# ecmwf/anemoi-graphs

Hardware: NVIDIA B200
Metric: O1280->ico7 graph edges/sec (CutOff encoder + MultiScale processor + KNN-3 decoder + EdgeLength/EdgeDirection) (higher is better)
Workload: dtype f32 filter + f64 decisions, int32 indices

## Files before the change

anemoi_graphs_b200/_build.py:

```python

from __future__ import annotations

import os
import shutil
import subprocess
import sys
from pathlib import Path

PKG = Path(__file__).resolve().parent
CSRC = PKG / "csrc"
LIB_DIR = PKG / "lib"
LIB_PATH = LIB_DIR / "libagx_b200.so"
OBJ_DIR = LIB_DIR / "obj"
SOURCES = ["agx_util.cu", "agx_index.cu", "agx_knn.cu", "agx_radius.cu", "agx_attrs.cu", "agx_mesh.cu", "agx_hex.cu", "agx_voronoi.cu", "agx_concat.cu", "agx_postprocess.cu"]
NVCC_FLAGS = [
    "-gencode", "arch=compute_100a,code=sm_100a",
    "-lineinfo", "-O3", "-std=c++17",
    "-Xcompiler", "-fPIC",
    "-Xcompiler", "-fvisibility=default",
]
LINK_FLAGS = ["-gencode", "arch=compute_100a,code=sm_100a", "--shared", "-cudart", "static"]


def find_nvcc() -> str:
    for cand in (os.environ.get("NVCC"), shutil.which("nvcc"), "/usr/local/cuda/bin/nvcc"):
        if cand and Path(cand).exists():
            return cand
    raise RuntimeError("nvcc not found (set NVCC=/path/to/nvcc)")


def is_stale() -> bool:
    if not LIB_PATH.exists():
        return True
    built = LIB_PATH.stat().st_mtime
    deps = [CSRC / s for s in SOURCES] + list(CSRC.glob("*.cuh")) + [PKG.parent / "include" / "agx_b200.h"]
    return any(d.stat().st_mtime > built for d in deps)


def build(force: bool = False, verbose: bool = False) -> Path:
    if not force and not is_stale():
        return LIB_PATH
    LIB_DIR.mkdir(exist_ok=True)
    OBJ_DIR.mkdir(exist_ok=True)
    nvcc = find_nvcc()
    headers = list(CSRC.glob("*.cuh")) + [PKG.parent / "include" / "agx_b200.h"]
    newest_header = max(h.stat().st_mtime for h in headers)
    jobs = []
    for src in SOURCES:
        obj = OBJ_DIR / (src + ".o")
        if not force and obj.exists() and obj.stat().st_mtime > max((CSRC / src).stat().st_mtime, newest_header):
            continue
        cmd = [nvcc, *NVCC_FLAGS, "-c", "-o", str(obj), str(CSRC / src)]
        if verbose:
            cmd[1:1] = ["-Xptxas", "-v"]
            print(" ".join(cmd))
        jobs.append((src, subprocess.Popen(cmd, stdout=subprocess.PIPE, stderr=subprocess.PIPE, text=True)))
    for src, proc in jobs:
        out, err = proc.communicate()
        if proc.returncode != 0:
            for _, other in jobs:
                if other.poll() is None:
                    other.kill()
            raise RuntimeError(f"nvcc failed on {src}:\n{out}\n{err}")
        if verbose:
            print(err)
    tmp = LIB_PATH.with_suffix(".so.tmp")
    cmd = [nvcc, *LINK_FLAGS, "-o", str(tmp), *[str(OBJ_DIR / (s + ".o")) for s in SOURCES]]
    res = subprocess.run(cmd, capture_output=True, text=True)
    if res.returncode != 0:
        raise RuntimeError(f"link failed:\n{res.stdout}\n{res.stderr}")
    os.replace(tmp, LIB_PATH)
    return LIB_PATH


if __name__ == "__main__":
    path = build(force="--force" in sys.argv, verbose="-v" in sys.argv)
    print(path)
```

anemoi_graphs_b200/_cabi.py:

```python

from __future__ import annotations

import ctypes
from ctypes import POINTER, c_char_p, c_double, c_int, c_int32, c_int64, c_void_p
from pathlib import Path

import torch

LIB_PATH = Path(__file__).resolve().parent / "lib" / "libagx_b200.so"

ABI_VERSION = 3
AGX_OK = 0
AGX_ERR_CUDA = -1
AGX_ERR_ARG = -2
AGX_ERR_UNSUPPORTED = -3
AGX_ERR_OVERFLOW = -4

NORM_CODES = {None: 0, "l1": 1, "l2": 2, "unit-max": 3, "unit-range": 4, "unit-std": 5}

SIGNATURES = {
    "agx_last_error": (c_char_p, []),
    "agx_abi_version": (c_int, []),
    "agx_launch_count": (c_int64, []),
    "agx_index_build": (c_int, [c_void_p, c_int64, c_int, c_int, c_double, c_void_p, POINTER(c_void_p)]),
    "agx_index_free": (c_int, [c_void_p, c_void_p]),
    "agx_index_info": (c_int, [c_void_p, POINTER(c_int64), POINTER(c_int)]),
    "agx_search_vectors": (c_int, [c_void_p, c_int64, c_void_p, c_void_p]),
    "agx_knn": (
        c_int,
        [c_void_p, c_void_p, c_int64, c_int, c_double, c_void_p, c_void_p, c_int64, c_void_p, c_void_p, c_void_p],
    ),
    "agx_knn_flagged": (
        c_int,
        [c_void_p, c_void_p, c_int64, c_int, c_double, c_void_p, c_void_p, c_int64, c_void_p, c_void_p, c_void_p, c_void_p],
    ),
    "agx_knn_redecide": (c_int, [c_void_p, c_void_p, c_int64, c_int, c_double, c_void_p, c_void_p, c_void_p]),
    "agx_knn_redecide_ranked": (
        c_int,
        [c_void_p, c_void_p, c_int64, c_int, c_double, c_void_p, c_void_p, c_void_p, c_void_p, c_void_p],
    ),
    "agx_knn_redecide_list": (
        c_int,
        [c_void_p, c_void_p, c_int64, c_int, c_double, c_void_p, c_void_p, c_void_p, c_void_p, c_void_p, c_void_p],
    ),
    "agx_compact_flags": (c_int, [c_void_p, c_int64, c_void_p, c_void_p, c_void_p]),
    "agx_set_query_order_mode": (None, [c_int]),
    "agx_last_query_order": (c_int, []),
    "agx_radius_count": (c_int, [c_void_p, c_void_p, c_int64, c_double, c_void_p, c_void_p]),
    "agx_exclusive_scan": (c_int, [c_void_p, c_int64, c_void_p, POINTER(c_int64), c_void_p]),
    "agx_radius_fill": (c_int, [c_void_p, c_void_p, c_int64, c_double, c_void_p, c_void_p, c_void_p, c_int64, c_void_p, c_void_p]),
    "agx_max_positive": (c_int, [c_void_p, c_int64, POINTER(c_double), POINTER(c_int64), c_void_p]),
    "agx_host_reference_rdist": (c_int, [c_void_p, c_void_p, c_int64, c_int, POINTER(c_double)]),
    "agx_order_resolve": (c_int, [c_void_p, c_void_p, c_int64, c_void_p, c_void_p, c_void_p, c_void_p, c_void_p]),
    "agx_gate_supported": (c_int, []),
    "agx_gate_wait": (c_int, [c_void_p, c_void_p]),
    "agx_gate_open": (c_int, [c_void_p, c_void_p]),
    "agx_mark_nodes": (c_int, [c_void_p, c_int64, c_int64, c_void_p, c_void_p]),
    "agx_relabel_nodes": (c_int, [c_void_p, c_int64, c_void_p, c_void_p]),
    "agx_restrict_flags": (
        c_int,
        [c_void_p, c_void_p, c_int64, c_void_p, c_int64, c_void_p, c_int64, c_void_p, c_void_p, c_double, c_void_p, c_void_p],
    ),
    "agx_sort_edges": (c_int, [c_void_p, c_void_p, c_int64, c_int64, c_int64, c_int, c_void_p, c_void_p]),
    "agx_gather_edge_columns": (
        c_int,
        [c_int, POINTER(c_void_p), POINTER(c_void_p), POINTER(c_int64), c_void_p, c_int64, c_void_p],
    ),
    "agx_set_output_maps": (None, [c_void_p, c_void_p]),
    "agx_concat_edges": (
        c_int,
        [c_void_p, c_void_p, c_int64, c_void_p, c_void_p, c_int64, c_int64, c_int64, c_void_p, POINTER(c_int64), c_void_p],
    ),
    "agx_relabel_rows": (c_int, [POINTER(c_void_p), POINTER(c_int64), c_int, c_void_p, c_void_p]),
    "agx_node_tables": (c_int, [c_void_p, c_int64, c_void_p, c_void_p, c_void_p]),
    "agx_edge_attrs": (
        c_int,
        [c_void_p, c_void_p, c_int64, c_void_p, c_void_p, c_void_p, c_void_p, c_int, c_int, c_void_p, c_int, c_int,
         c_void_p, c_void_p, c_int, c_void_p],
    ),
    "agx_edge_attrs_workspace": (c_int64, []),
    "agx_edge_attrs_stats": (
        c_int,
        [c_void_p, c_void_p, c_int64, c_void_p, c_void_p, c_void_p, c_void_p, c_int, c_int, c_int, c_void_p, c_void_p,
         c_void_p, c_void_p, c_void_p],
    ),
    "agx_edge_attrs_stats_flagged": (
        c_int,
        [c_void_p, c_void_p, c_int64, c_void_p, c_void_p, c_void_p, c_void_p, c_int, c_int, c_int, c_void_p, c_void_p,
         c_void_p, c_void_p, c_void_p, c_int, c_int, c_void_p],
    ),
    "agx_edge_attrs_stats_list": (
        c_int,
        [c_void_p, c_void_p, c_int64, c_int, c_void_p, c_void_p, c_void_p, c_void_p, c_void_p, c_void_p, c_int, c_int,
         c_int, c_void_p, c_void_p, c_void_p, c_void_p, c_void_p],
    ),
    "agx_edge_attrs_apply": (
        c_int,
        [c_void_p, c_void_p, c_int64, c_void_p, c_void_p, c_void_p, c_void_p, c_int, c_int, c_void_p, c_int, c_int,
         c_void_p, c_void_p, c_int, c_int64, c_int, c_void_p, c_void_p],
    ),
    "agx_icosphere": (c_int, [c_int, c_void_p, c_void_p, c_void_p, c_void_p]),
    "agx_multiscale_tri_count": (
        c_int,
        [c_int, c_void_p, POINTER(c_int32), c_int, c_int, c_void_p, c_void_p, c_void_p, c_void_p, c_void_p],
    ),
    "agx_multiscale_scratch_per_node": (c_int64, [c_int, c_int]),
    "agx_multiscale_tri_count_mapped": (
        c_int,
        [c_int, c_void_p, POINTER(c_int32), c_int, c_int, c_int64, c_void_p, c_void_p, c_void_p, c_void_p, c_void_p],
    ),
    "agx_multiscale_tri_fill": (c_int, [c_int64, c_void_p, c_void_p, c_void_p, c_int64, c_void_p, c_void_p, c_void_p]),
    "agx_voronoi_areas": (
        c_int,
        [c_void_p, c_int64, c_void_p, c_int, c_int, c_void_p, c_int64, c_double, c_void_p, c_void_p, c_void_p],
    ),
    "agx_voronoi_areas_small": (c_int, [c_void_p, c_int64, c_void_p, c_int64, c_double, c_void_p, c_void_p, c_void_p]),
    "agx_healpix_nodes": (c_int, [c_int, c_void_p, c_void_p]),
    "agx_hex_num_cells": (c_int64, [c_int]),
    "agx_hex_cells": (c_int, [c_int, c_void_p, c_void_p, c_void_p]),
    "agx_hex_adjacency": (c_int, [c_void_p, c_void_p, c_int64, c_void_p, c_void_p, c_void_p]),
    "agx_multiscale_adj_count": (
        c_int,
        [c_int, POINTER(c_void_p), POINTER(c_void_p), POINTER(c_void_p), POINTER(c_void_p), c_int, c_int, c_int64,
         c_void_p, c_void_p, c_void_p],
    ),
}

_lib = None


class AgxError(RuntimeError):
    """A CUDA-side failure reported by libagx_b200."""


def load_library(path: Path | None = None) -> ctypes.CDLL:
    global _lib
    if _lib is not None and path is None:
        return _lib
    p = Path(path) if path is not None else LIB_PATH
    if not p.exists():
        raise RuntimeError(
            f"{p} is missing: the CUDA extension has not been built. Run `python -m anemoi_graphs_b200._build` "
            "(needs nvcc). This package has no CPU fallback."
        )
    lib = ctypes.CDLL(str(p))
    for name, (restype, argtypes) in SIGNATURES.items():
        fn = getattr(lib, name)
        fn.restype = restype
        fn.argtypes = argtypes
    if lib.agx_abi_version() != ABI_VERSION:
        raise RuntimeError(f"{p}: ABI version {lib.agx_abi_version()} != {ABI_VERSION}; rebuild the library")
    if path is None:
        _lib = lib
    return lib


def require_cuda() -> None:
    if not torch.cuda.is_available():
        raise RuntimeError(
            "anemoi_graphs_b200 needs a CUDA device (B200, sm_100a); there is no CPU fallback for the "
            "edge-construction path."
        )


def check(rc: int) -> None:
    if rc == AGX_OK:
        return
    msg = load_library().agx_last_error().decode(errors="replace")
    if rc == AGX_ERR_ARG:
        raise ValueError(msg)
    if rc == AGX_ERR_UNSUPPORTED:
        raise NotImplementedError(msg)
    raise AgxError(f"libagx_b200 error {rc}: {msg}")


def ptr(t: torch.Tensor | None) -> int | None:
    if t is None:
        return None
    assert t.is_cuda and t.is_contiguous(), "C-ABI buffers must be contiguous CUDA tensors"
    return t.data_ptr()


def current_stream() -> int:
    return torch.cuda.current_stream().cuda_stream


def launch_count() -> int:
    return int(load_library().agx_launch_count())
```

anemoi_graphs_b200/device.py:

```python

from __future__ import annotations

import contextlib
import os
from dataclasses import dataclass, field

import torch

from . import _cabi

_defer_depth = 0
_pending: list[torch.cuda.Event] = []
_works: dict[int, list] = {}
_resident = False


def set_resident(flag: bool) -> bool:
    global _resident
    prev, _resident = _resident, bool(flag)
    return prev


def is_resident() -> bool:
    return _resident
# ... 283 lines not shown
    st = NodeState(key=_key(x), x=upload_replicated(x))
    nodes[STATE_ATTR] = st
    return st


_upload_streams: dict = {}
_prefetch_events: list = []
PREFETCH_MIN_BYTES = 1 << 20


def prefetch_coordinates(nodes) -> None:
    if not torch.cuda.is_available() or sharded_output():
        return
    x = nodes.get("x", None) if hasattr(nodes, "get") else None
    if not isinstance(x, torch.Tensor) or x.is_cuda or x.dtype != torch.float32 or x.dim() != 2 or not x.is_pinned():
        return
    if x.numel() * x.element_size() < PREFETCH_MIN_BYTES or not x.is_contiguous():
        return
    st = nodes.get(STATE_ATTR, None)
    if isinstance(st, NodeState) and (st.prov is not None or st.key == _key(x)):
        return
    dev = compute_device()
    key = dev.index if dev.index is not None else torch.cuda.current_device()
    if key not in _upload_streams:
        _upload_streams[key] = torch.cuda.Stream(device=dev)
    side = _upload_streams[key]
    x_dev = torch.empty(x.shape, dtype=torch.float32, device=dev)
    side.wait_stream(torch.cuda.current_stream())
    with torch.cuda.stream(side):
        x_dev.copy_(x, non_blocking=True)
        uploaded = torch.cuda.Event()
        uploaded.record(side)
    x_dev.record_stream(side)
    st = NodeState(key=_key(x), x=x_dev)
    st.extras["uploaded"] = uploaded
    nodes[STATE_ATTR] = st
    _prefetch_events.append(uploaded)


SLICED_UPLOAD_MIN_BYTES = int(float(__import__("os").environ.get("AGX_SLICED_UPLOAD_MIN_BYTES", "4e6")))


def upload_replicated(x: torch.Tensor) -> torch.Tensor:
    if x.is_cuda or not sharded_output() or x.numel() * x.element_size() < SLICED_UPLOAD_MIN_BYTES:
        return to_device(x, torch.float32)
    import torch.distributed as dist

    if dist.get_backend() != "nccl":
        return to_device(x, torch.float32)
    rank, w = world()
    dev = compute_device()
    n = int(x.shape[0])
    per = (n + w - 1) // w
    full = torch.empty((per * w,) + tuple(x.shape[1:]), dtype=torch.float32, device=dev)
    lo, hi = min(rank * per, n), min((rank + 1) * per, n)
    if hi > lo:
        full[lo:hi].copy_(x[lo:hi], non_blocking=True)
    dist.all_gather_into_tensor(full, full[rank * per : (rank + 1) * per])
    return full[:n]


INDEX_CACHE_MAX_NODES = int(float(__import__("os").environ.get("AGX_INDEX_CACHE_MAX_NODES", "2e6")))


class _Borrowed:

    def __init__(self, index) -> None:
        self.index = index

    def __enter__(self):
        return self.index

    def __exit__(self, *exc) -> None:
        return None


def neighbour_index(st: NodeState | None, x: torch.Tensor, hint_k: int = 0, hint_radius: float = 0.0):
    from . import ops

    if st is None or x is not st.x or int(x.shape[0]) > INDEX_CACHE_MAX_NODES:
        return ops.NeighbourIndex(x, hint_k=hint_k, hint_radius=hint_radius)
    cache = st.extras.setdefault("index", {})
    key = (int(hint_k), float(hint_radius))
    hit = cache.get(key)
    if hit is None or hit.handle is None:
        hit = cache[key] = ops.NeighbourIndex(x, hint_k=hint_k, hint_radius=hint_radius)
    return _Borrowed(hit)


def seed_node_state(nodes, x_dev: torch.Tensor) -> NodeState:
    st = NodeState(key=_key(nodes["x"]), x=x_dev.contiguous())
    nodes[STATE_ATTR] = st
    return st


def node_tables(nodes, with_rotation: bool = True, provisional_ok: bool = False):
    from . import ops

    st = node_state(nodes, provisional_ok)
    if st.tables is None:
        st.tables = ops.NodeTables(st.x)
    return st.tables


_provisionals: list = []
_prov_seq = 0
SHARED_NODE_ORDER = __import__("os").environ.get("AGX_SHARED_ORDER", "1") != "0"
_order_pool = None
last_trace: dict = {}
LAZY_NODE_ORDER = __import__("os").environ.get("AGX_LAZY_ORDER", "1") != "0"


PIN_SORT_THREAD = __import__("os").environ.get("AGX_PIN_SORT", "auto")
_sort_thread_pinned = False


def _pin_sort_thread(follower: bool) -> None:
    global _sort_thread_pinned
    want = PIN_SORT_THREAD == "1" or (PIN_SORT_THREAD == "auto" and world()[1] > 1)
    if not want or _sort_thread_pinned or follower:
        return
    import os

    try:
        cpus = sorted(os.sched_getaffinity(0))
        local = int(os.environ.get("LOCAL_RANK", "0"))
        os.sched_setaffinity(0, {cpus[-1 - (local % len(cpus))]})
        _sort_thread_pinned = True
    except (AttributeError, OSError):
        pass


_upload_pool = None
UPLOAD_HANDOVER = os.environ.get("AGX_UPLOAD_HANDOVER", "0") == "1"


def _upload_helper():
    global _upload_pool
    if _upload_pool is None:
        from concurrent.futures import ThreadPoolExecutor

        _upload_pool = ThreadPoolExecutor(max_workers=1, thread_name_prefix="agx-order-upload")
    return _upload_pool


PRELAUNCH_TAIL = os.environ.get("AGX_PRELAUNCH_TAIL", "auto")


def _prelaunch_wanted() -> bool:
    mode = PRELAUNCH_TAIL
    if isinstance(mode, bool):
        return mode
    return mode == "1" or (mode == "auto" and _resident)


_gate_ring = None
_gate_next = 0
GATE_RING = 256


def _new_gates(count: int) -> torch.Tensor:
    global _gate_ring, _gate_next
    if _gate_ring is None:
        _gate_ring = torch.zeros(GATE_RING, dtype=torch.int32, pin_memory=True)
    if _gate_next % GATE_RING + count > GATE_RING:
        _gate_next += GATE_RING - _gate_next % GATE_RING
    lo = _gate_next % GATE_RING
    _gate_next += count
    gates = _gate_ring[lo : lo + count]
    gates.zero_()
    return gates


def _pool():
    global _order_pool
    if _order_pool is None:
        from concurrent.futures import ThreadPoolExecutor

        _order_pool = ThreadPoolExecutor(max_workers=1, thread_name_prefix="agx-node-order")
    return _order_pool


class Provisional:

    def __init__(self, x_prov: torch.Tensor, sorter, combine) -> None:
        import time

        self.x_prov = x_prov.contiguous()
        n = int(x_prov.shape[0])
        self.n = n
        dev = x_prov.device
        self.combine = combine
        self.x_final = torch.empty((n, 2), dtype=torch.float32, device=dev)
        self.x_host = None
        self.order_host = host_tensor((n,), torch.int64)
        self.order_dev = torch.empty(n, dtype=torch.int64, device=dev)
        self.rank = torch.empty(n + 1, dtype=torch.int64, device=dev)
        self.rows: list = []
        self.fixups: list = []
        self.finalizers: list = []
        self.nodes = None
        self.state = None
        self.on_resolved = None
        self.done = False
        self._order_ready = None
        columns = self.x_prov.t().contiguous()
        staged = torch.empty((2, n), dtype=torch.float32, pin_memory=True)
        ready = torch.cuda.Event()
        ready.record()
        side = _copy_stream(dev)
        with torch.cuda.stream(side):
            side.wait_event(ready)
            staged.copy_(columns, non_blocking=True)
            copied = torch.cuda.Event()
            copied.record(side)
        columns.record_stream(side)
        self.trace = {"created": time.perf_counter()}
        max_parts = 2
        group, prov_seq = None, 0
        if SHARED_NODE_ORDER and world()[1] > 1:
            from . import shm

            group = shm.local_group()
        if group is not None:
            global _prov_seq
            global _shared_host_used
            _shared_host_used = True
            prov_seq, _prov_seq = _prov_seq, _prov_seq + 1
            parts_pinned = shm.arena().tensor((max_parts, n), torch.int64)
            stamps = group.order[prov_seq % shm.RING]
        else:
            parts_pinned = torch.empty((max_parts, n), dtype=torch.int64, pin_memory=True)
        parts_dev = torch.empty((max_parts, n), dtype=torch.int64, device=dev)
        follower = group is not None and group.rank != 0
        ostream = _order_stream(dev)
        for t in (parts_dev, self.order_dev, self.rank, self.x_final, self.x_prov):
            t.record_stream(ostream)
        import threading

        gates = None
        if _prelaunch_wanted() and combine == "latlon" and _cabi.load_library().agx_gate_supported():
            gates = _new_gates(max_parts)
        gates_np = gates.numpy() if gates is not None else None
        self._gates, self._parts_pinned, self._parts_dev, self._group = gates, parts_pinned, parts_dev, group
        self._coords_ready = threading.Event()

        def work():
            from ._cabi import check, load_library

            torch.cuda.set_device(dev)
            _pin_sort_thread(follower)
            self.trace["worker_start"] = time.perf_counter()
            copied.synchronize()
            self._coords_ready.set()
            self.trace["coords_on_host"] = time.perf_counter()
            cols = staged.numpy()
            sent = []

            def upload(i: int, part) -> None:
                if part is not None:
                    parts_pinned[i].numpy()[:] = part
                    if group is not None:
                        stamps[i] = prov_seq + 1
                        group.wake_followers()
                if gates_np is not None:
                    gates_np[i] = 1
                    return
                with torch.cuda.stream(ostream):
                    parts_dev[i].copy_(parts_pinned[i], non_blocking=True)

            handed_over = []

            def emit(part) -> None:
                i = len(sent)
                self.trace[f"part{i}_ready"] = time.perf_counter()
                if i < max_parts:
                    if UPLOAD_HANDOVER and part is not None and i + 1 < max_parts:
                        handed_over.append(_upload_helper().submit(upload, i, part))
                    else:
                        for f in handed_over:
                            f.result()
                        upload(i, part)
                sent.append(part)
                self.trace[f"part{i}_sent"] = time.perf_counter()

            if follower:
                from . import shm

                t_start = time.perf_counter()
                t_first = None
                for i in range(max_parts):
                    if i == 0 or t_first is None:
                        group.sleep_until_woken()
                    else:
                        time.sleep(max(0.0, 0.8 * t_first - (time.perf_counter() - t_prev)))
                        while int(stamps[i]) not in (prov_seq + 1, -(prov_seq + 1)):
                            time.sleep(0)
                        group.drain_wakeups()
                    if int(stamps[i]) == -(prov_seq + 1):
                        raise RuntimeError("the rank that sorts the node order failed; see its traceback")
                    shm._spin(lambda i=i: int(stamps[i]) == prov_seq + 1, f"part {i} of node order {prov_seq}")
                    t_prev = time.perf_counter()
                    if i == 0:
                        t_first = t_prev - t_start
                    emit(None)
                out = (None, None)
            else:
                try:
                    out = sorter(cols[0], cols[1], emit)
                except BaseException:
                    if group is not None:
                        stamps[:] = -(prov_seq + 1)
                        for _ in range(max_parts):
                            group.wake_followers()
                    raise
                out = out if isinstance(out, tuple) else (out,)
            self.trace["sorted"] = time.perf_counter()
            if gates_np is not None:
                if len(sent) != max_parts:
                    raise RuntimeError(f"node order: the sorter emitted {len(sent)} index arrays, {max_parts} were queued for")
                return None
            if self.combine == "latlon" and len(out) == 2 and len(sent) == 2:
                check(
                    load_library().agx_order_resolve(
                        parts_dev[0].data_ptr(), parts_dev[1].data_ptr(), n, self.x_prov.data_ptr(),
                        self.x_final.data_ptr(), self.order_dev.data_ptr(), self.rank.data_ptr(), ostream.cuda_stream,
                    )
                )
                done = torch.cuda.Event()
                done.record(ostream)
                self._order_ready = done
                if group is not None:
                    _pending.append(done)
                self.trace["order_launched"] = time.perf_counter()
                return None
            assert not follower, "a shared node order needs the 'latlon' combine"
            return out

        def guarded():
            try:
                return work()
            except BaseException:
                self._coords_ready.set()
                if gates_np is not None:
                    import numpy as np

                    parts_pinned.numpy()[:] = np.arange(n, dtype=np.int64)
                    gates_np[:] = 1
                raise

        self.future = _pool().submit(guarded)
        _provisionals.append(self)

    def __getstate__(self):
        return {"done": True, "n": self.n}

    def attach(self, nodes, state: NodeState) -> None:
        self.nodes, self.state = nodes, state
        state.prov = self
        state.x = self.x_prov

    def add_row(self, tensor: torch.Tensor, row: int, host_row: torch.Tensor | None, cols: tuple | None = None) -> None:
        self.rows.append((tensor, row, host_row, cols))

    def add_fixup(self, fn) -> None:
        self.fixups.append(fn)

    def add_finalizer(self, fn) -> None:
        self.finalizers.append(fn)

    def resolve(self) -> None:
        if self.done:
            return
        self.done = True
        if self in _provisionals:
            _provisionals.remove(self)
        import time

        self.trace["resolve_enter"] = time.perf_counter()
        dev = self.x_prov.device
        order_dev, rank = self.order_dev, self.rank
        gated = self._gates is not None
        if gated:
            from ._cabi import check, load_library

            lib = load_library()
            self._coords_ready.wait()
            main = torch.cuda.current_stream()
            for i in range(int(self._gates.numel())):
                check(lib.agx_gate_wait(self._gates.data_ptr() + 4 * i, main.cuda_stream))
                self._parts_dev[i].copy_(self._parts_pinned[i], non_blocking=True)
            if self._group is not None:
                uploaded = torch.cuda.Event()
                uploaded.record(main)
                _pending.append(uploaded)
            check(
                lib.agx_order_resolve(
                    self._parts_dev[0].data_ptr(), self._parts_dev[1].data_ptr(), self.n, self.x_prov.data_ptr(),
                    self.x_final.data_ptr(), order_dev.data_ptr(), rank.data_ptr(), main.cuda_stream,
                )
            )
            self.trace["order_launched"] = time.perf_counter()
        else:
            parts = self.future.result()
            self.trace["resolve_got_order"] = time.perf_counter()
        if gated:
            pass
        elif parts is None:
            torch.cuda.current_stream().wait_event(self._order_ready)
        else:
            staged = torch.empty((len(parts), self.n), dtype=torch.int64, pin_memory=True)
            for i, part in enumerate(parts):
                staged[i].numpy()[:] = part
            parts_dev = staged.to(dev, non_blocking=True)
            order_dev = self.combine(*[parts_dev[i] for i in range(int(parts_dev.shape[0]))]).contiguous()
            rank[order_dev] = torch.arange(self.n, dtype=torch.int64, device=dev)
            torch.index_select(self.x_prov, 0, order_dev, out=self.x_final)
        self.order_dev = order_dev
        self.rank = rank
        fixups, self.fixups = self.fixups, []
        for fn in fixups:
            fn(self)
        from . import ops

        for tensor, row, host_row, cols in self.rows:
            wait_for(tensor)
        main = torch.cuda.current_stream()
        side = _order_stream(dev)
        fixed = torch.cuda.Event()
        fixed.record(main)
        with torch.cuda.stream(side):
            side.wait_event(fixed)
            ops.relabel_rows([tensor[row] for tensor, row, host_row, cols in self.rows], rank)
            relabelled = torch.cuda.Event()
            relabelled.record(side)
        for tensor, row, host_row, cols in self.rows:
            tensor.record_stream(side)
        rank.record_stream(side)
        finalizers, self.finalizers = self.finalizers, []
        for fn in finalizers:
            fn(self)
        main.wait_event(relabelled)
        for tensor, row, host_row, cols in self.rows:
            if host_row is not None and host_row.numel():
                to_host_into(tensor[row] if cols is None else tensor[row, cols[0] : cols[1]], host_row)
        self.rows = []
        copy_replicated_to_host(order_dev, self.order_host)
        if self.x_host is not None:
            copy_replicated_to_host(self.x_final, self.x_host)
        if gated:
            self.trace["tail_queued"] = time.perf_counter()
            self.future.result()
            self.trace["resolve_got_order"] = time.perf_counter()
        if self.state is not None:
            st = self.state
            st.prov = None
            st.x = self.x_final
            st.tables = None
            st.extras = {}
            if self.nodes is not None:
                st.key = _key(self.nodes["x"])
        if self.on_resolved is not None:
            self.on_resolved(self)
        self.trace["resolve_done"] = time.perf_counter()
        global last_trace
        last_trace = self.trace


def active_provisional(nodes):
    st = nodes.get(STATE_ATTR, None) if hasattr(nodes, "get") else None
    return st.prov if isinstance(st, NodeState) else None


class EdgeMeta:
    __slots__ = ("prov", "fixup", "local", "tie_flags", "tie_list", "regular_k", "shard", "flag_base", "regular_targets")

    def __init__(self) -> None:
        self.prov = (None, None)
        self.fixup = None
        self.tie_flags = None
        self.tie_list = None
        self.regular_k = 0
        self.regular_targets = False
        self.flag_base = 0
        self.shard = None
        self.local = None


_edge_meta: dict[int, tuple] = {}


def edge_meta(edge_index: torch.Tensor, create: bool = False) -> EdgeMeta | None:
    import weakref

    key = id(edge_index)
    hit = _edge_meta.get(key)
    if hit is not None and hit[0]() is edge_index:
        return hit[1]
    if not create:
        return None
    meta = EdgeMeta()
    _edge_meta[key] = (weakref.ref(edge_index, lambda _r, key=key: _edge_meta.pop(key, None)), meta)
    return meta


def tag_rows(edge_index: torch.Tensor, src_prov, dst_prov) -> torch.Tensor:
    if src_prov is not None or dst_prov is not None:
        edge_meta(edge_index, create=True).prov = (src_prov, dst_prov)
    return edge_index


def row_tags(edge_index: torch.Tensor) -> tuple:
    meta = edge_meta(edge_index)
    tags = meta.prov if meta is not None else (None, None)
    return tuple(p if (p is not None and not p.done) else None for p in tags)


def edge_shard(edge_index: torch.Tensor) -> Shard | None:
    meta = edge_meta(edge_index)
    return meta.shard if meta is not None else None


EARLY_TARGET_ROW = os.environ.get("AGX_EARLY_TARGET_ROW", "1") != "0"
_early_rows: dict = {}


def emit_regular_target_row(n_targets: int, k: int) -> None:
    e = int(n_targets) * int(k)
    if not EARLY_TARGET_ROW or e <= 0 or e >= 2**31 or (n_targets, k) in _early_rows or sharded_output():
        return
    dev = compute_device()
    host = torch.empty((2, e), dtype=torch.int32, pin_memory=True)
    row = torch.div(torch.arange(e, dtype=torch.int32, device=dev), int(k), rounding_mode="floor")
    side = _copy_stream(dev)
    for uploaded in _prefetch_events:
        side.wait_event(uploaded)
    to_host_into(row, host[1])
    _early_rows[(int(n_targets), int(k))] = host


def _adopt_early_row(edge_dev: torch.Tensor) -> torch.Tensor | None:
    meta = edge_meta(edge_dev)
    if not _early_rows or meta is None or not meta.regular_targets or not meta.regular_k or edge_dev.dtype != torch.int32:
        return None
    return _early_rows.pop((int(edge_dev.shape[1]) // meta.regular_k, meta.regular_k), None)


def edge_index_like_input(edge_dev: torch.Tensor, reference_input: torch.Tensor) -> torch.Tensor:
    tags = row_tags(edge_dev)
    shard = edge_shard(edge_dev)
    if shard is not None and not (shard.world > 1 and sharded_output()):
        shard = None
    if tags == (None, None):
        early = _adopt_early_row(edge_dev) if (shard is None and not reference_input.is_cuda) else None
        if early is None:
            return like_input(edge_dev, reference_input, shard, dim=1)
        to_host_into(edge_dev[0], early[0])
        return early
    if reference_input.is_cuda:
        for row, prov in enumerate(tags):
            if prov is not None:
                prov.add_row(edge_dev, row, None)
        return edge_dev
    early = None
    if shard is None:
        if tags[1] is None:
            early = _adopt_early_row(edge_dev)
        out = early if early is not None else torch.empty(edge_dev.shape, dtype=edge_dev.dtype, pin_memory=True)
        lo, hi, cols = 0, int(edge_dev.shape[1]), None
    else:
        out = host_tensor((2, shard.total), edge_dev.dtype, require_shared=True)
        if shard.replicated:
            lo, hi = shard_range(int(edge_dev.shape[1]), shard.rank, shard.world)
            cols = (lo, hi)
        else:
            lo, hi, cols = shard.offset, shard.offset + int(edge_dev.shape[1]), None
    for row, prov in enumerate(tags):
        host_row = out[row, lo:hi]
        if prov is None:
            if row == 1 and early is not None:
                continue
            if hi > lo:
                to_host_into(edge_dev[row] if cols is None else edge_dev[row, cols[0] : cols[1]], host_row)
        else:
            prov.add_row(edge_dev, row, host_row, cols)
    return out


def remember_edge_index(store, host_or_dev: torch.Tensor, dev: torch.Tensor) -> None:
    store[EDGE_ATTR] = (_key(host_or_dev), dev)


def device_edge_index(store) -> torch.Tensor:
    ei = store["edge_index"]
    if ei.is_cuda:
        return ei if ei.dtype == torch.int32 and ei.is_contiguous() else ei.to(torch.int32).contiguous()
    cached = store.get(EDGE_ATTR, None) if hasattr(store, "get") else None
    if cached is not None and cached[0] == _key(ei):
        return cached[1]
    flush()
    dev = to_device(ei, torch.int32)
    remember_edge_index(store, ei, dev)
    return dev


# ... 406 lines not shown
```

anemoi_graphs_b200/generate/tri_icosahedron.py:

```python

from __future__ import annotations

import numpy as np
import torch

from .. import device as _device
from .. import ops


class DeviceMesh:

    def __init__(self, icosphere: ops.Icosphere, order_dev: torch.Tensor) -> None:
        self.icosphere = icosphere
        self.order_dev = order_dev

    def number_of_nodes(self) -> int:
        return int(self.order_dev.shape[0])

    def __getstate__(self):
        return {"icosphere": None, "order_dev": None}


def get_icosphere(resolution: int) -> ops.Icosphere:
    return ops.Icosphere(int(resolution))


def get_latlon_coords_icosphere(resolution: int) -> np.ndarray:
    return get_icosphere(resolution).latlon.cpu().numpy()


def _ordering_of(latlon_dev: torch.Tensor) -> torch.Tensor:
    lat_dev = latlon_dev[:, 0].contiguous()
    lon = latlon_dev[:, 1].contiguous().cpu().numpy()
    index_latitude = torch.from_numpy(np.argsort(lon)).to(latlon_dev.device)
    lat_sorted = lat_dev[index_latitude].cpu().numpy()
    index_longitude = torch.from_numpy(np.argsort(lat_sorted)).to(latlon_dev.device)
    return index_latitude[index_longitude.flip(0)]


def _sort_columns_host(lat: np.ndarray, lon: np.ndarray, emit=None):
    index_latitude = np.argsort(lon)
    if emit is not None:
        emit(index_latitude)
    index_longitude = np.argsort(lat[index_latitude])
    if emit is not None:
        emit(index_longitude)
    return index_latitude, index_longitude


def _combine_order(index_latitude: torch.Tensor, index_longitude: torch.Tensor) -> torch.Tensor:
    return index_latitude[index_longitude.flip(0)]


def create_tri_nodes_provisional(resolution: int):
    ico = get_icosphere(resolution)
    mesh = DeviceMesh(ico, None)
    prov = _device.Provisional(ico.latlon, _sort_columns_host, "latlon")
    prov.on_resolved = lambda p: setattr(mesh, "order_dev", p.order_dev)
    return mesh, prov


def create_tri_nodes(resolution: int, area_mask_builder=None):
    ico = get_icosphere(resolution)
    node_ordering = _ordering_of(ico.latlon)

    if area_mask_builder is not None:
        area_mask = area_mask_builder.get_mask_device(ico.latlon)
        node_ordering = node_ordering[area_mask[node_ordering]]

    return DeviceMesh(ico, node_ordering), ico.latlon, node_ordering


def create_stretched_tri_nodes(base_resolution: int, lam_resolution: int, area_mask_builder=None):
    assert area_mask_builder is not None, "AOI mask builder must be provided to build refined grid."
    lam = get_icosphere(lam_resolution)
    if base_resolution <= lam_resolution:
        base_latlon = lam.latlon[: ops.ico_num_vertices(base_resolution)]
    else:
        base_latlon = get_icosphere(base_resolution).latlon
    base_area_mask = ~area_mask_builder.get_mask_device(base_latlon)
    lam_area_mask = area_mask_builder.get_mask_device(lam.latlon)

    coords_rad = torch.cat([base_latlon[base_area_mask], lam.latlon[lam_area_mask]])
    node_ordering = _ordering_of(coords_rad)
    return DeviceMesh(lam, node_ordering), coords_rad, node_ordering


def multiscale_edges(
    nodes, resolutions, x_hops: int = 1, area_mask_builder=None, allow_provisional: bool = False
) -> torch.Tensor:
    assert x_hops > 0, "x_hops == 0, graph would have no edges ..."
    resolutions = [int(r) for r in resolutions]
    mesh = nodes.get("_nx_graph", None)
    ico = mesh.icosphere if isinstance(mesh, DeviceMesh) and mesh.icosphere is not None else None
    if ico is None or ico.max_level < max(resolutions):
        ico = get_icosphere(max(resolutions))
    node_type = nodes["node_type"]
    st = _device.node_state(nodes, provisional_ok=(allow_provisional and node_type == "TriNodes" and area_mask_builder is None))
    n_nodes = int(st.x.shape[0])
    if node_type == "TriNodes" and area_mask_builder is None and n_nodes == ops.ico_num_vertices(ico.max_level):
        if st.prov is not None:
            identity = torch.arange(n_nodes, dtype=torch.int32, device=st.x.device)
            edges = ops.multiscale_tri_edges(ico, resolutions, x_hops, identity)
            return _device.tag_rows(edges, st.prov, st.prov)
        mesh = nodes.get("_nx_graph", None)
        if isinstance(mesh, DeviceMesh) and mesh.order_dev is not None:
            order = mesh.order_dev
        else:
            order = torch.as_tensor(np.asarray(nodes["_node_ordering"]))
        return ops.multiscale_tri_edges(ico, resolutions, x_hops, order)
    if st.prov is not None:
        st = _device.node_state(nodes)
    nv = ops.ico_num_vertices(max(resolutions))
    coords = ico.latlon[:nv]
    with ops.NeighbourIndex(st.x, hint_k=1) as index:
        nearest = index.knn(coords, 1, tag="knn_vertex_map")[0]
    if area_mask_builder is not None:
        valid = area_mask_builder.get_mask_device(coords)
        vertex_map = torch.where(valid, nearest, torch.full_like(nearest, -1))
    else:
        vertex_map = nearest
    if ico.max_level > max(resolutions):
        pad = torch.full((ops.ico_num_vertices(ico.max_level) - nv,), -1, dtype=torch.int32, device=vertex_map.device)
        vertex_map = torch.cat([vertex_map, pad])
    return ops.multiscale_tri_edges_mapped(ico, resolutions, x_hops, n_nodes, vertex_map)
```

include/agx_b200.h:

```cpp
#ifndef AGX_B200_H
#define AGX_B200_H

#include <stdint.h>

#ifdef __cplusplus
extern "C" {
#endif

#define AGX_ABI_VERSION 3

#define AGX_OK 0
#define AGX_ERR_CUDA -1
#define AGX_ERR_ARG -2
#define AGX_ERR_UNSUPPORTED -3
#define AGX_ERR_OVERFLOW -4

#define AGX_NORM_NONE 0
#define AGX_NORM_L1 1
#define AGX_NORM_L2 2
#define AGX_NORM_UNIT_MAX 3
#define AGX_NORM_UNIT_RANGE 4
#define AGX_NORM_UNIT_STD 5

typedef struct agx_index agx_index_t;

const char* agx_last_error(void);
int agx_abi_version(void);
int64_t agx_launch_count(void);

int agx_index_build(const float* latlon , int64_t n, int cells_per_face, int hint_k,
                    double hint_radius, void* stream, agx_index_t** out);
int agx_index_free(agx_index_t* index, void* stream);
int agx_index_info(const agx_index_t* index, int64_t* n, int* cells_per_face);
int agx_search_vectors(const float* latlon , int64_t n, float* xyz , void* stream);

int agx_knn(const agx_index_t* index, const float* q_latlon , int64_t nq, int k, double max_radius,
            int32_t* out_src , int32_t* out_dst , int64_t dst_base,
            double* out_rdist , int64_t* stats , void* stream);

int agx_knn_flagged(const agx_index_t* index, const float* q_latlon , int64_t nq, int k, double max_radius,
                    int32_t* out_src , int32_t* out_dst , int64_t dst_base,
                    double* out_rdist , int64_t* stats , uint8_t* tie_flags ,
                    void* stream);

int agx_knn_redecide(const agx_index_t* index, const float* q_latlon , int64_t nq, int k, double max_radius,
                     int32_t* out_src , const uint8_t* tie_flags , void* stream);

int agx_knn_redecide_list(const agx_index_t* index, const float* q_latlon , int64_t nq, int k,
                          double max_radius, int32_t* out_src , const int32_t* list ,
                          const int64_t* count , const int64_t* rank ,
                          const int64_t* order , void* stream);
int agx_compact_flags(const uint8_t* flags , int64_t n, int32_t* list ,
                      int64_t* count , void* stream);
int agx_knn_redecide_ranked(const agx_index_t* index, const float* q_latlon , int64_t nq, int k,
                            double max_radius, int32_t* out_src ,
                            const uint8_t* tie_flags , const int64_t* rank ,
                            const int64_t* order , void* stream);

void agx_set_query_order_mode(int mode);
int agx_last_query_order(void);

int agx_radius_count(const agx_index_t* index, const float* q_latlon , int64_t nq, double radius,
                     int32_t* counts , void* stream);
int agx_exclusive_scan(const int32_t* counts , int64_t n, int64_t* offsets ,
                       int64_t* total , void* stream);
int agx_radius_fill(const agx_index_t* index, const float* q_latlon , int64_t nq, double radius,
                    const int64_t* offsets , int32_t* out_src , int32_t* out_dst ,
                    int64_t dst_base, int64_t* stats , void* stream);

int agx_max_positive(const double* values , int64_t n, double* out_value ,
                     int64_t* out_index , void* stream);
int agx_host_reference_rdist(const float* q_latlon , const float* nb_latlon ,
                             int64_t n_cand, int n_nb, double* out_rdist );

int agx_mark_nodes(const int32_t* row , int64_t n, int64_t n_nodes, int32_t* flags , void* stream);
int agx_relabel_nodes(int32_t* row , int64_t n, const int64_t* new_index , void* stream);
int agx_relabel_rows(int32_t* const* rows , const int64_t* lens , int n_rows,
                     const int64_t* new_index , void* stream);

int agx_restrict_flags(const int32_t* edge_src , const int32_t* edge_dst , int64_t n_edges,
                       const float* src_latlon , int64_t n_src_nodes, const float* dst_latlon ,
                       int64_t n_dst_nodes, const uint8_t* src_mask ,
                       const uint8_t* dst_mask , double max_radius, uint8_t* keep ,
                       void* stream);
int agx_sort_edges(const int32_t* key_row , const int32_t* other_row , int64_t n_edges,
                   int64_t n_key_nodes, int64_t n_other_nodes, int descending, int32_t* perm , void* stream);
int agx_gather_edge_columns(int n_arrays, const void* const* src ,
                            void* const* dst , const int64_t* row_bytes ,
                            const int32_t* index , int64_t n_index, void* stream);

void agx_set_output_maps(const int64_t* src_map , const int64_t* dst_map );

int agx_concat_edges(const int32_t* a_src , const int32_t* a_dst, int64_t na, const int32_t* b_src ,
                     const int32_t* b_dst, int64_t nb, int64_t n_src_nodes, int64_t n_dst_nodes,
                     int32_t* out , int64_t* n_unique , void* stream);

int agx_order_resolve(const int64_t* index_latitude , const int64_t* index_longitude , int64_t n,
                      const float* x_in , float* x_out , int64_t* order ,
                      int64_t* rank , void* stream);

int agx_gate_supported(void);
int agx_gate_wait(const uint32_t* gate , void* stream);
int agx_gate_open(uint32_t* gate , void* stream);

int agx_node_tables(const float* latlon , int64_t n, float* src_rec ,
                    double* dst_rec , void* stream);
int agx_edge_attrs(const int32_t* edge_src , const int32_t* edge_dst , int64_t n_edges,
                   const float* src_rec , const float* src_latlon ,
                   const double* dst_rec , const float* dst_latlon ,
                   int len_norm , int len_invert, float* out_len ,
                   int dir_norm , int dir_rotated, float* out_dir ,
                   double* workspace ,
                   int regular_k ,
                   void* stream);
int64_t agx_edge_attrs_workspace(void);
int agx_edge_attrs_stats(const int32_t* edge_src, const int32_t* edge_dst, int64_t n_edges, const float* src_rec,
                         const float* src_latlon, const double* dst_rec, const float* dst_latlon, int want_len,
                         int want_dir, int dir_rotated, float* out_len ,
                         float* out_dir , double* stats , double* workspace, void* stream);
int agx_edge_attrs_stats_flagged(const int32_t* edge_src, const int32_t* edge_dst, int64_t n_edges,
                                 const float* src_rec, const float* src_latlon, const double* dst_rec,
                                 const float* dst_latlon, int want_len, int want_dir, int dir_rotated, float* out_len,
                                 float* out_dir, double* stats , double* workspace,
                                 const uint8_t* dst_flags , int flag_mode, int regular_k, void* stream);
int agx_edge_attrs_stats_list(const int32_t* edge_src, const int32_t* edge_dst, int64_t n_edges, int regular_k,
                              const int32_t* list , const int64_t* count , const float* src_rec,
                              const float* src_latlon, const double* dst_rec, const float* dst_latlon, int want_len,
                              int want_dir, int dir_rotated, float* out_len, float* out_dir, double* stats ,
                              double* workspace, void* stream);
int agx_edge_attrs_apply(const int32_t* edge_src, const int32_t* edge_dst, int64_t n_edges, const float* src_rec,
                         const float* src_latlon, const double* dst_rec, const float* dst_latlon, int len_norm,
                         int len_invert, float* out_len, int dir_norm, int dir_rotated, float* out_dir,
                         const double* stats , int n_stat_sets,
                         int64_t n_edges_global, int raw_present, double* workspace, void* stream);

int agx_icosphere(int max_level, double* vertices , int32_t* faces_all ,
                  float* latlon , void* stream);
int agx_multiscale_tri_count(int max_level, const int32_t* faces_all , const int32_t* levels ,
                             int n_levels, int x_hops, const int32_t* node_ordering ,
                             const int32_t* rank_of_vertex , int32_t* counts ,
                             int32_t* scratch , void* stream);
int64_t agx_multiscale_scratch_per_node(int n_levels, int x_hops);
int agx_multiscale_tri_count_mapped(int max_level, const int32_t* faces_all , const int32_t* levels ,
                                    int n_levels, int x_hops, int64_t n_nodes, const int32_t* vertex_map ,
                                    const int32_t* node_vertex , int32_t* counts ,
                                    int32_t* scratch , void* stream);
int agx_multiscale_tri_fill(int64_t n_nodes, const int32_t* counts, const int64_t* offsets ,
                            const int32_t* scratch, int64_t scratch_per_node, int32_t* out_src,
                            int32_t* out_dst, void* stream);

int64_t agx_hex_num_cells(int res);
int agx_hex_cells(int res, double* latlon , uint8_t* pentagon , void* stream);
int agx_hex_adjacency(const int32_t* knn7 , const uint8_t* pentagon , int64_t n,
                      int32_t* nb , int32_t* deg , void* stream);
int agx_multiscale_adj_count(int n_levels, const int32_t* const* nb ,
                             const int32_t* const* deg, const int32_t* const* cell_node,
                             const int32_t* const* node_cell, int x_hops, int walk_all, int64_t n_nodes,
                             int32_t* counts , int32_t* scratch , void* stream);

int agx_healpix_nodes(int resolution , float* latlon , void* stream);

int agx_voronoi_areas(const float* latlon , int64_t n, const int32_t* knn , int k, int exhaustive,
                      const int32_t* subset , int64_t m, double radius, double* areas ,
                      int32_t* status , void* stream);
int agx_voronoi_areas_small(const float* latlon , int64_t n, const int32_t* subset , int64_t m,
                            double radius, double* areas , int32_t* status , void* stream);

#ifdef __cplusplus
}
#endif
#endif
```

Before: 6.041 billion.

## Run host node-order argsort on a native C++ thread with numpy's argsort

```diff
diff --git a/anemoi_graphs_b200/_build.py b/anemoi_graphs_b200/_build.py
--- a/anemoi_graphs_b200/_build.py
+++ b/anemoi_graphs_b200/_build.py
@@ -12,7 +12,9 @@
 LIB_DIR = PKG / "lib"
 LIB_PATH = LIB_DIR / "libagx_b200.so"
 OBJ_DIR = LIB_DIR / "obj"
-SOURCES = ["agx_util.cu", "agx_index.cu", "agx_knn.cu", "agx_radius.cu", "agx_attrs.cu", "agx_mesh.cu", "agx_hex.cu", "agx_voronoi.cu", "agx_concat.cu", "agx_postprocess.cu"]
+NPSORT_SOURCE = CSRC / "agx_npsort.cpp"
+NPSORT_PATH = LIB_DIR / "libagx_npsort.so"
+SOURCES = ["agx_util.cu", "agx_index.cu", "agx_knn.cu", "agx_radius.cu", "agx_attrs.cu", "agx_mesh.cu", "agx_hex.cu", "agx_voronoi.cu", "agx_concat.cu", "agx_postprocess.cu", "agx_order.cu"]
 NVCC_FLAGS = [
     "-gencode", "arch=compute_100a,code=sm_100a",
     "-lineinfo", "-O3", "-std=c++17",
@@ -29,7 +31,7 @@
     raise RuntimeError("nvcc not found (set NVCC=/path/to/nvcc)")
 
 
-def is_stale() -> bool:
+def _lib_stale() -> bool:
     if not LIB_PATH.exists():
         return True
     built = LIB_PATH.stat().st_mtime
@@ -37,10 +39,40 @@
     return any(d.stat().st_mtime > built for d in deps)
 
 
+def _npsort_stale() -> bool:
+    return not NPSORT_PATH.exists() or NPSORT_SOURCE.stat().st_mtime > NPSORT_PATH.stat().st_mtime
+
+
+def is_stale() -> bool:
+    return _lib_stale() or _npsort_stale()
+
+
+def build_npsort() -> Path:
+    import sysconfig
+
+    import numpy
+
+    cxx = os.environ.get("CXX") or shutil.which("c++") or shutil.which("g++")
+    if not cxx:
+        raise RuntimeError("no C++ compiler found for libagx_npsort.so (set CXX)")
+    tmp = NPSORT_PATH.with_suffix(".so.tmp")
+    cmd = [cxx, "-O2", "-std=c++17", "-shared", "-fPIC", "-I" + sysconfig.get_paths()["include"],
+           "-I" + numpy.get_include(), "-o", str(tmp), str(NPSORT_SOURCE)]
+    res = subprocess.run(cmd, capture_output=True, text=True)
+    if res.returncode != 0:
+        raise RuntimeError(f"{cxx} failed on {NPSORT_SOURCE.name}:\n{res.stdout}\n{res.stderr}")
+    os.replace(tmp, NPSORT_PATH)
+    return NPSORT_PATH
+
+
 def build(force: bool = False, verbose: bool = False) -> Path:
     if not force and not is_stale():
         return LIB_PATH
     LIB_DIR.mkdir(exist_ok=True)
+    if force or _npsort_stale():
+        build_npsort()
+    if not force and not _lib_stale():
+        return LIB_PATH
     OBJ_DIR.mkdir(exist_ok=True)
     nvcc = find_nvcc()
     headers = list(CSRC.glob("*.cuh")) + [PKG.parent / "include" / "agx_b200.h"]
diff --git a/anemoi_graphs_b200/_cabi.py b/anemoi_graphs_b200/_cabi.py
--- a/anemoi_graphs_b200/_cabi.py
+++ b/anemoi_graphs_b200/_cabi.py
@@ -55,6 +55,10 @@
     "agx_gate_supported": (c_int, []),
     "agx_gate_wait": (c_int, [c_void_p, c_void_p]),
     "agx_gate_open": (c_int, [c_void_p, c_void_p]),
+    "agx_order_sort_set_argsort": (c_int, [c_void_p]),
+    "agx_order_sort_submit": (c_int, [c_void_p, c_int64, c_void_p, c_void_p, c_void_p, c_int, c_int, POINTER(c_int64)]),
+    "agx_order_sort_wait": (c_int, [c_int64, c_int, POINTER(c_double)]),
+    "agx_order_sort_shutdown": (None, []),
     "agx_mark_nodes": (c_int, [c_void_p, c_int64, c_int64, c_void_p, c_void_p]),
     "agx_relabel_nodes": (c_int, [c_void_p, c_int64, c_void_p, c_void_p]),
     "agx_restrict_flags": (
@@ -155,6 +159,18 @@
     return lib
 
 
+NPSORT_PATH = LIB_PATH.parent / "libagx_npsort.so"
+
+
+def numpy_argsort_float32() -> int | None:
+    if not NPSORT_PATH.exists():
+        return None
+    fn = ctypes.PyDLL(str(NPSORT_PATH)).agx_numpy_argsort_float32
+    fn.restype = c_void_p
+    fn.argtypes = []
+    return fn() or None
+
+
 def require_cuda() -> None:
     if not torch.cuda.is_available():
         raise RuntimeError(
diff --git a/anemoi_graphs_b200/csrc/agx_npsort.cpp b/anemoi_graphs_b200/csrc/agx_npsort.cpp
--- /dev/null
+++ b/anemoi_graphs_b200/csrc/agx_npsort.cpp
@@ -0,0 +1,19 @@
+#define PY_SSIZE_T_CLEAN
+#include <Python.h>
+#define NPY_NO_DEPRECATED_API NPY_1_7_API_VERSION
+#include <numpy/arrayobject.h>
+
+extern "C" void* agx_numpy_argsort_float32(void) {
+    if (_import_array() < 0) {
+        PyErr_Clear();
+        return nullptr;
+    }
+    PyArray_Descr* descr = PyArray_DescrFromType(NPY_FLOAT32);
+    if (!descr) {
+        PyErr_Clear();
+        return nullptr;
+    }
+    void* fn = (void*)PyDataType_GetArrFuncs(descr)->argsort[NPY_QUICKSORT];
+    Py_DECREF(descr);
+    return fn;
+}
diff --git a/anemoi_graphs_b200/csrc/agx_order.cu b/anemoi_graphs_b200/csrc/agx_order.cu
--- /dev/null
+++ b/anemoi_graphs_b200/csrc/agx_order.cu
@@ -0,0 +1,199 @@
+#include <string.h>
+#include <time.h>
+
+#include <condition_variable>
+#include <deque>
+#include <mutex>
+#include <thread>
+#include <unordered_map>
+#include <vector>
+
+#include "agx_common.cuh"
+
+typedef int (*agx_argsort_f32)(void* values, int64_t* idx, int64_t n, void* unused);
+
+namespace {
+
+double now_s() {
+    timespec ts;
+    clock_gettime(CLOCK_MONOTONIC, &ts);
+    return (double)ts.tv_sec + 1e-9 * (double)ts.tv_nsec;
+}
+
+struct Job {
+    const float* cols;
+    int64_t n;
+    int64_t* parts;
+    uint32_t* gates;
+    cudaEvent_t copied;
+    int device;
+    int fail_at;
+    int stage = 0;
+    int status = AGX_OK;
+    char error[256] = "";
+    double marks[AGX_ORDER_MARKS] = {0};
+};
+
+struct Sorter {
+    std::mutex mu;
+    std::condition_variable work_cv, done_cv;
+    std::deque<Job*> queue;
+    std::unordered_map<int64_t, Job*> jobs;
+    int64_t next_id = 1;
+    bool stop = false;
+    std::thread* thread = nullptr;
+    agx_argsort_f32 argsort = nullptr;
+    std::vector<float> gathered;
+};
+
+Sorter& sorter() {
+    static Sorter* s = new Sorter();
+    return *s;
+}
+
+void set_stage(Sorter& s, Job* job, int stage, int slot) {
+    job->marks[slot] = now_s();
+    std::lock_guard<std::mutex> lock(s.mu);
+    job->stage = stage;
+    s.done_cv.notify_all();
+}
+
+void open_gate(Job* job, int i) {
+    if (job->gates) __atomic_store_n(&job->gates[i], 1u, __ATOMIC_RELEASE);
+}
+
+int sort_into(Sorter& s, const float* values, int64_t* idx, int64_t n) {
+    for (int64_t i = 0; i < n; ++i) idx[i] = i;
+    return s.argsort(const_cast<float*>(values), idx, n, nullptr);
+}
+
+void fail(Job* job, int opened, const char* fmt, const char* what) {
+    job->status = AGX_ERR_CUDA;
+    snprintf(job->error, sizeof(job->error), fmt, what);
+    for (int i = opened; i < 2; ++i) {
+        for (int64_t v = 0; v < job->n; ++v) job->parts[i * job->n + v] = v;
+        open_gate(job, i);
+    }
+}
+
+void run(Sorter& s, Job* job) {
+    const int64_t n = job->n;
+    job->marks[AGX_ORDER_MARK_START] = now_s();
+    int current = -1;
+    if (job->device >= 0 && (cudaGetDevice(&current) != cudaSuccess || current != job->device)) {
+        cudaError_t err = cudaSetDevice(job->device);
+        if (err != cudaSuccess) {
+            fail(job, 0, "node order: cudaSetDevice failed: %s", cudaGetErrorString(err));
+            set_stage(s, job, 2, AGX_ORDER_MARK_DONE);
+            return;
+        }
+    }
+    cudaError_t err = job->copied ? cudaEventSynchronize(job->copied) : cudaSuccess;
+    set_stage(s, job, 1, AGX_ORDER_MARK_COORDS);
+    if (err != cudaSuccess) {
+        cudaGetLastError();
+        fail(job, 0, "node order: waiting for the coordinate copy failed: %s", cudaGetErrorString(err));
+        set_stage(s, job, 2, AGX_ORDER_MARK_DONE);
+        return;
+    }
+    const float* lat = job->cols;
+    const float* lon = job->cols + n;
+    int64_t* part0 = job->parts;
+    int64_t* part1 = job->parts + n;
+    if (job->fail_at == 1 || sort_into(s, lon, part0, n) != 0) {
+        fail(job, 0, "node order: %s failed", "the argsort of the longitudes");
+        set_stage(s, job, 2, AGX_ORDER_MARK_DONE);
+        return;
+    }
+    job->marks[AGX_ORDER_MARK_PART0] = now_s();
+    open_gate(job, 0);
+    if ((int64_t)s.gathered.size() < n) s.gathered.resize(n);
+    float* gathered = s.gathered.data();
+    for (int64_t i = 0; i < n; ++i) gathered[i] = lat[part0[i]];
+    if (job->fail_at == 2 || sort_into(s, gathered, part1, n) != 0) {
+        fail(job, 1, "node order: %s failed", "the argsort of the gathered latitudes");
+        set_stage(s, job, 2, AGX_ORDER_MARK_DONE);
+        return;
+    }
+    job->marks[AGX_ORDER_MARK_PART1] = now_s();
+    open_gate(job, 1);
+    set_stage(s, job, 2, AGX_ORDER_MARK_DONE);
+}
+
+void loop() {
+    Sorter& s = sorter();
+    for (;;) {
+        Job* job = nullptr;
+        {
+            std::unique_lock<std::mutex> lock(s.mu);
+            s.work_cv.wait(lock, [&] { return s.stop || !s.queue.empty(); });
+            if (s.queue.empty()) return;
+            job = s.queue.front();
+            s.queue.pop_front();
+        }
+        run(s, job);
+    }
+}
+
+}
+
+extern "C" int agx_order_sort_set_argsort(void* argsort_f32) {
+    AGX_REQUIRE(argsort_f32, AGX_ERR_ARG, "agx_order_sort_set_argsort: NULL function");
+    Sorter& s = sorter();
+    std::lock_guard<std::mutex> lock(s.mu);
+    s.argsort = (agx_argsort_f32)argsort_f32;
+    return AGX_OK;
+}
+
+extern "C" int agx_order_sort_submit(const float* cols, int64_t n, int64_t* parts, uint32_t* gates, void* copied,
+                                     int device, int fail_at, int64_t* job_id) {
+    AGX_REQUIRE(cols && parts && job_id && n >= 0, AGX_ERR_ARG, "agx_order_sort_submit: NULL buffer or n < 0");
+    AGX_REQUIRE(!gates || ((uintptr_t)gates & 3) == 0, AGX_ERR_ARG, "agx_order_sort_submit: unaligned gate words");
+    Sorter& s = sorter();
+    std::lock_guard<std::mutex> lock(s.mu);
+    AGX_REQUIRE(s.argsort, AGX_ERR_ARG, "agx_order_sort_submit: no argsort set (agx_order_sort_set_argsort)");
+    AGX_REQUIRE(!s.stop, AGX_ERR_ARG, "agx_order_sort_submit: the sorting thread has been shut down");
+    if (!s.thread) s.thread = new std::thread(loop);
+    Job* job = new Job();
+    job->cols = cols;
+    job->n = n;
+    job->parts = parts;
+    job->gates = gates;
+    job->copied = (cudaEvent_t)copied;
+    job->device = device;
+    job->fail_at = fail_at;
+    int64_t id = s.next_id++;
+    s.jobs[id] = job;
+    s.queue.push_back(job);
+    s.work_cv.notify_one();
+    *job_id = id;
+    return AGX_OK;
+}
+
+extern "C" int agx_order_sort_wait(int64_t job_id, int stage, double* marks) {
+    Sorter& s = sorter();
+    std::unique_lock<std::mutex> lock(s.mu);
+    auto it = s.jobs.find(job_id);
+    AGX_REQUIRE(it != s.jobs.end(), AGX_ERR_ARG, "agx_order_sort_wait: unknown job %lld", (long long)job_id);
+    Job* job = it->second;
+    s.done_cv.wait(lock, [&] { return job->stage >= (stage >= 2 ? 2 : 1); });
+    if (stage < 2) return AGX_OK;
+    if (marks) memcpy(marks, job->marks, sizeof(job->marks));
+    int rc = job->status;
+    if (rc != AGX_OK) agx_set_error("%s", job->error);
+    s.jobs.erase(it);
+    delete job;
+    return rc;
+}
+
+extern "C" void agx_order_sort_shutdown(void) {
+    Sorter& s = sorter();
+    std::thread* t = nullptr;
+    {
+        std::lock_guard<std::mutex> lock(s.mu);
+        s.stop = true;
+        t = s.thread;
+        s.work_cv.notify_all();
+    }
+    if (t && t->joinable()) t->join();
+}
diff --git a/anemoi_graphs_b200/device.py b/anemoi_graphs_b200/device.py
--- a/anemoi_graphs_b200/device.py
+++ b/anemoi_graphs_b200/device.py
@@ -459,6 +459,41 @@
     if isinstance(mode, bool):
         return mode
     return mode == "1" or (mode == "auto" and _resident)
+
+
+NATIVE_SORT = os.environ.get("AGX_NATIVE_SORT", "auto")
+_native_sort_state = None
+_native_fail_at = 0
+_native_jobs: dict = {}
+
+
+def _native_sort_mode(sorter, group, combine) -> str | None:
+    global _native_sort_state
+    mode = NATIVE_SORT
+    if mode is False or mode == "0" or group is not None or combine != "latlon":
+        return None
+    from .generate import tri_icosahedron
+
+    if not getattr(sorter, "has_native_equivalent", False):
+        return None
+    if mode == "auto" and not _prelaunch_wanted():
+        return None
+    if _native_sort_state is None:
+        import atexit
+
+        fn = _cabi.numpy_argsort_float32()
+        if fn is None:
+            if mode is True or mode == "1":
+                raise RuntimeError("AGX_NATIVE_SORT=1: numpy's float32 argsort cannot be looked up (libagx_npsort.so)")
+            _native_sort_state = False
+            return None
+        lib = _cabi.load_library()
+        _cabi.check(lib.agx_order_sort_set_argsort(fn))
+        atexit.register(lib.agx_order_sort_shutdown)
+        _native_sort_state = "unchecked"
+    if _native_sort_state is False:
+        return None
+    return "verify" if _native_sort_state == "unchecked" else "on"
 
 
 _gate_ring = None
@@ -545,11 +580,28 @@
             t.record_stream(ostream)
         import threading
 
+        native = _native_sort_mode(sorter, group, combine)
         gates = None
-        if _prelaunch_wanted() and combine == "latlon" and _cabi.load_library().agx_gate_supported():
+        if _prelaunch_wanted() and combine == "latlon" and native != "verify" and _cabi.load_library().agx_gate_supported():
             gates = _new_gates(max_parts)
         gates_np = gates.numpy() if gates is not None else None
         self._gates, self._parts_pinned, self._parts_dev, self._group = gates, parts_pinned, parts_dev, group
+        self._native_job = None
+        if native is not None:
+            from ctypes import c_int64
+
+            job = c_int64(0)
+            _cabi.check(
+                _cabi.load_library().agx_order_sort_submit(
+                    staged.data_ptr(), n, parts_pinned.data_ptr(), None if gates is None else gates.data_ptr(),
+                    copied.cuda_event, dev.index if dev.index is not None else torch.cuda.current_device(),
+                    _native_fail_at, job,
+                )
+            )
+            self._native_job, self._native_verify, self._staged = job.value, native == "verify", staged
+            _native_jobs[job.value] = (staged, parts_pinned, gates, copied)
+            _provisionals.append(self)
+            return
         self._coords_ready = threading.Event()
 
         def work():
@@ -659,6 +711,38 @@
         self.future = _pool().submit(guarded)
         _provisionals.append(self)
 
+    def _finish_native_sort(self) -> None:
+        from ctypes import c_double
+
+        from ._cabi import check, load_library
+
+        marks = (c_double * 5)()
+        job, self._native_job = self._native_job, None
+        rc = load_library().agx_order_sort_wait(job, 2, marks)
+        _native_jobs.pop(job, None)
+        start, coords, part0, part1, done = marks
+        self.trace.update(worker_start=start, coords_on_host=coords, sorted=done)
+        if part0:
+            self.trace.update(part0_ready=part0, part0_sent=part0)
+        if part1:
+            self.trace.update(part1_ready=part1, part1_sent=part1)
+        check(rc)
+        if self._native_verify:
+            import warnings
+
+            import numpy as np
+
+            global _native_sort_state
+            cols, parts = self._staged.numpy(), self._parts_pinned.numpy()
+            index_latitude = np.argsort(cols[1])
+            index_longitude = np.argsort(cols[0][index_latitude])
+            if np.array_equal(parts[0], index_latitude) and np.array_equal(parts[1], index_longitude):
+                _native_sort_state = True
+            else:
+                warnings.warn("node order: the native argsort differs from np.argsort; using the Python sorting thread")
+                _native_sort_state = False
+                parts[0], parts[1] = index_latitude, index_longitude
+
     def __getstate__(self):
         return {"done": True, "n": self.n}
 
@@ -688,11 +772,15 @@
         dev = self.x_prov.device
         order_dev, rank = self.order_dev, self.rank
         gated = self._gates is not None
+        native = self._native_job is not None
         if gated:
             from ._cabi import check, load_library
 
             lib = load_library()
-            self._coords_ready.wait()
+            if native:
+                check(lib.agx_order_sort_wait(self._native_job, 1, None))
+            else:
+                self._coords_ready.wait()
             main = torch.cuda.current_stream()
             for i in range(int(self._gates.numel())):
                 check(lib.agx_gate_wait(self._gates.data_ptr() + 4 * i, main.cuda_stream))
@@ -708,6 +796,21 @@
                 )
             )
             self.trace["order_launched"] = time.perf_counter()
+        elif native:
+            self._finish_native_sort()
+            ostream = _order_stream(dev)
+            with torch.cuda.stream(ostream):
+                self._parts_dev.copy_(self._parts_pinned, non_blocking=True)
+                _cabi.check(
+                    _cabi.load_library().agx_order_resolve(
+                        self._parts_dev[0].data_ptr(), self._parts_dev[1].data_ptr(), self.n, self.x_prov.data_ptr(),
+                        self.x_final.data_ptr(), order_dev.data_ptr(), rank.data_ptr(), ostream.cuda_stream,
+                    )
+                )
+                self._order_ready = torch.cuda.Event()
+                self._order_ready.record(ostream)
+            parts = None
+            self.trace["resolve_got_order"] = time.perf_counter()
         else:
             parts = self.future.result()
             self.trace["resolve_got_order"] = time.perf_counter()
@@ -757,7 +860,10 @@
             copy_replicated_to_host(self.x_final, self.x_host)
         if gated:
             self.trace["tail_queued"] = time.perf_counter()
-            self.future.result()
+            if native:
+                self._finish_native_sort()
+            else:
+                self.future.result()
             self.trace["resolve_got_order"] = time.perf_counter()
         if self.state is not None:
             st = self.state
diff --git a/anemoi_graphs_b200/generate/tri_icosahedron.py b/anemoi_graphs_b200/generate/tri_icosahedron.py
--- a/anemoi_graphs_b200/generate/tri_icosahedron.py
+++ b/anemoi_graphs_b200/generate/tri_icosahedron.py
@@ -46,6 +46,9 @@
     if emit is not None:
         emit(index_longitude)
     return index_latitude, index_longitude
+
+
+_sort_columns_host.has_native_equivalent = True
 
 
 def _combine_order(index_latitude: torch.Tensor, index_longitude: torch.Tensor) -> torch.Tensor:
diff --git a/include/agx_b200.h b/include/agx_b200.h
--- a/include/agx_b200.h
+++ b/include/agx_b200.h
@@ -103,6 +103,19 @@
 int agx_gate_wait(const uint32_t* gate , void* stream);
 int agx_gate_open(uint32_t* gate , void* stream);
 
+#define AGX_ORDER_MARK_START 0
+#define AGX_ORDER_MARK_COORDS 1
+#define AGX_ORDER_MARK_PART0 2
+#define AGX_ORDER_MARK_PART1 3
+#define AGX_ORDER_MARK_DONE 4
+#define AGX_ORDER_MARKS 5
+int agx_order_sort_set_argsort(void* argsort_f32);
+int agx_order_sort_submit(const float* cols , int64_t n, int64_t* parts ,
+                          uint32_t* gates , void* copied , int device,
+                          int fail_at, int64_t* job_id );
+int agx_order_sort_wait(int64_t job_id, int stage, double* marks );
+void agx_order_sort_shutdown(void);
+
 int agx_node_tables(const float* latlon , int64_t n, float* src_rec ,
                     double* dst_rec , void* stream);
 int agx_edge_attrs(const int32_t* edge_src , const int32_t* edge_dst , int64_t n_edges,
```

Result: faster. 6.309 billion (median of 6 runs) (+4.4%).
